# AllenNeuralDynamics/aind-exaspim-neuron-segmentation

Measured on AMD Instinct MI355X. Metric: affinity voxels/sec on 96^3 patches over a 1024x1024x1024 volume, 1 MI355X, higher is better.
Workload: dtype fp16; 1 GPU; 1024x1024x1024 uint16 volume, 96^3 patches, overlap 32, trim 8, batch 16, fp16 (IEEE half) storage of activations and weights / fp32 accumulate (BASELINE.json configs[2]); streams=1

## Files before the change

### aind_exaspim_neuron_segmentation_amd/_native.py

```python

import ctypes
import os

_HERE = os.path.dirname(os.path.abspath(__file__))
LIB_PATH = os.path.join(_HERE, "csrc", "libexaspim_affinity.so")

DT_F32, DT_BF16, DT_F16 = 0, 1, 2
VOX_U8, VOX_U16, VOX_I16, VOX_F32, VOX_F64 = 0, 1, 2, 3, 4
IN_F32, IN_PADDED_F32, IN_PADDED_SPLIT_F16, IN_PADDED_SPLIT_BF16 = 0, 1, 2, 3
UP_CONVT = 0x100
OPT_SEPARATE_POOL, OPT_SEPARATE_DEEP_POOLS, OPT_PLAIN_UPSAMPLE, OPT_FIRST_PER_GROUP = 1, 2, 4, 8
OPT_UPSAMPLE_PER_THREAD = 16

DTYPE_CODES = {
    "fp32": DT_F32, "float32": DT_F32, "f32": DT_F32,
    "bf16": DT_BF16, "bfloat16": DT_BF16,
    "fp16": DT_F16, "float16": DT_F16, "f16": DT_F16,
}


class Block(ctypes.Structure):

    _fields_ = [
        ("dims", ctypes.c_int32 * 3),
        ("origin", ctypes.c_int32 * 3),
        ("global_", ctypes.c_int32 * 3),
    ]

    @classmethod
    def make(cls, dims, origin=None, global_shape=None):
        origin = (0, 0, 0) if origin is None else origin
        global_shape = dims if global_shape is None else global_shape
        b = cls()
        b.dims[:] = [int(v) for v in dims]
        b.origin[:] = [int(v) for v in origin]
        b.global_[:] = [int(v) for v in global_shape]
        return b


class Window(ctypes.Structure):

    _fields_ = [
        ("patch", ctypes.c_int32 * 3),
        ("overlap", ctypes.c_int32 * 3),
        ("trim", ctypes.c_int32),
    ]

    @classmethod
    def make(cls, patch, overlap, trim):
        w = cls()
        w.patch[:] = [int(v) for v in patch]
        w.overlap[:] = [int(v) for v in overlap]
        w.trim = int(trim)
        return w


_lib = None

_I32x5 = ctypes.c_int32 * 5
_I32x3 = ctypes.c_int32 * 3
_vp = ctypes.c_void_p
_sz = ctypes.c_size_t
_i32 = ctypes.c_int32

SIGNATURES = {
# ... 86 lines not shown
```

### aind_exaspim_neuron_segmentation_amd/csrc/common.h

```cpp
#pragma once

#include <hip/hip_runtime.h>

#include <cstdarg>
#include <cstddef>
#include <cstdint>
#include <cstdio>

#include "../../include/exaspim_affinity.h"

namespace exaspim {

void set_error(const char* fmt, ...);
const char* get_error();

#define EXA_CHECK_ARG(cond, ...)                 \
    do {                                         \
        if (!(cond)) {                           \
            ::exaspim::set_error(__VA_ARGS__);   \
            return EXASPIM_E_INVALID;            \
        }                                        \
    } while (0)

#define EXA_CHECK_HIP(expr)                                                  \
// ... 68 lines not shown
    int cin_real = 0, cin = 0;
    int cout_real = 0, cout = 0;
    size_t w_off = 0;
    size_t b_off = 0;
    size_t p_off = 0;
};

struct UNetPlan {
    int channels[5] = {0, 0, 0, 0, 0};
    int out_channels = 0;
    int dtype = 0;
    bool convt = false;
    ConvTLayer up[4];
    int c0 = 0, c0p = 0;
    size_t first_p_off = 0;
    size_t first_w_off = 0;
    size_t first_b_off = 0;
    ConvLayer conv[kNumMfmaConvs];
    size_t head_p_off = 0;
    size_t head_w_off = 0;
    size_t head_b_off = 0;
    size_t packed_bytes = 0;
    size_t n_params = 0;
};

bool make_plan(const int32_t channels[5], int32_t out_channels, int32_t dtype,
               UNetPlan* plan);

int pack_weights(const UNetPlan& plan, const float* params, void* packed_host);

struct ConvArgs {
    const void* src_a;
    const void* src_b;
    int ca, cb;
    const void* weights;
    const void* weights_paired = nullptr;
    const void* weights_k32 = nullptr;
    const float* bias;
    void* dst;
    int cout;
    int n, d, h, w;
    float slope;
    const float* head_w = nullptr;
    const float* head_b = nullptr;
    float* head_out = nullptr;
    int head_oc = 0;
    int head_sigmoid = 0;
    int org[3] = {0, 0, 0};
    int ext[3] = {0, 0, 0};
    void* pool_dst = nullptr;
    float* partial = nullptr;
    size_t partial_patch_bytes = 0;
    int ksplit = 1;
#ifdef EXASPIM_TRACE
    unsigned long long* trace = nullptr;
#endif
};

int launch_conv3x3x3(int dtype, const ConvArgs& a, hipStream_t stream);
int launch_conv3x3x3_thin(int dtype, const ConvArgs& a, hipStream_t stream);
int conv_zcol_main_extent(int ext, int axis);
bool conv_can_fuse_head(int cout, int w, int head_oc);
bool conv_can_fuse_pool(int dtype, int cout, int d, int h, int w);

int launch_conv_first(int dtype, const float* x, float* xpad, const float* w, const float* bias,
                      void* dst, int n, int d, int h, int wd, int c0p, float slope,
                      hipStream_t stream, bool first_no_strips = false);
int launch_convt2(int dtype, const void* src, const void* weights, const float* bias, void* dst,
                  int n, int d, int h, int w, int cin, int cout, hipStream_t stream);
int launch_maxpool2(int dtype, const void* src, void* dst, int n, int d, int h, int w,
                    int c, hipStream_t stream);
int launch_upsample2(int dtype, const void* src, void* dst, int n, int d, int h, int w,
                     int c, int margin, hipStream_t stream, bool plain_kernel = false, bool per_thread = false);
int launch_absmax(int dtype, const void* src, size_t bytes, float* out, hipStream_t stream);
int launch_head(int dtype, const void* src, const float* w, const float* bias,
                float* out, int n, int d, int h, int wd, int c0p, int out_channels,
                int apply_sigmoid, hipStream_t stream);

}
```

### aind_exaspim_neuron_segmentation_amd/csrc/conv3d.hip

```cpp

#include <cstdlib>
#include <type_traits>

#include "common.h"

namespace exaspim {

typedef float f32x16 __attribute__((ext_vector_type(16)));
typedef float f32x4 __attribute__((ext_vector_type(4)));
typedef __bf16 bf16x8 __attribute__((ext_vector_type(8)));
typedef _Float16 f16x8 __attribute__((ext_vector_type(8)));

typedef unsigned int u32x4_t __attribute__((ext_vector_type(4)));

struct F32Tag { static constexpr int kG = 4; static constexpr int kCode = EXASPIM_DT_F32; };
struct BF16Tag { static constexpr int kG = 8; static constexpr int kCode = EXASPIM_DT_BF16; };
struct F16Tag { static constexpr int kG = 8; static constexpr int kCode = EXASPIM_DT_F16; };

template <typename Tag>
__device__ __forceinline__ void mma(f32x16& acc, const uint4& wf, const uint4& xf);

template <>
__device__ __forceinline__ void mma<F32Tag>(f32x16& acc, const uint4& wf, const uint4& xf) {
    acc = __builtin_amdgcn_mfma_f32_32x32x2f32(__uint_as_float(wf.x), __uint_as_float(xf.x), acc, 0, 0, 0);
// ... 1047 lines not shown
#if EXASPIM_BUFFER_STORES & 4
                    const __amdgpu_buffer_rsrc_t prsrc = make_rsrc(pplane, (size_t)CPT * pvox * 32);
#endif
#pragma unroll
                    for (int p0 = 0; p0 < NP; p0 += 64) {
                        const int p = p0 + lane_e;
#if EXASPIM_BUFFER_STORES & 4
                        const bool live0 = p < NP;
                        const int pc = live0 ? p : 0;
                        const int zp = pc / (8 * CPT * 2), rem = pc % (8 * CPT * 2);
                        const int ck = rem / 16, xp = (rem % 16) >> 1, sb = rem & 1;
                        const bool live = live0 && zb + 2 * zp + 1 < TZ;
                        const int zr = zb + 2 * zp + 1 < TZ ? zp : 0;
                        {
                            const char* rec = wl + (2 * zr) * (32 * RECP) + (2 * xp) * RECP + (ck * 2 + sb) * 16;
#else
                        const int zp = p / (8 * CPT * 2), rem = p % (8 * CPT * 2);
                        const int ck = rem / 16, xp = (rem % 16) >> 1, sb = rem & 1;
                        if (p < NP && zb + 2 * zp + 1 < TZ) {
                            const char* rec = wl + (2 * zp) * (32 * RECP) + (2 * xp) * RECP + (ck * 2 + sb) * 16;
#endif
                            uint4 m = *reinterpret_cast<const uint4*>(rec);
                            if (ES == 2) m = key16(m);
#pragma unroll
                            for (int k = 1; k < 8; ++k) {
                                const uint4 v = *reinterpret_cast<const uint4*>(
                                    rec + (k >> 2) * (32 * RECP) + ((k >> 1) & 1) * 16 * RECP + (k & 1) * RECP);
                                m = ES == 2 ? maxkey16(m, key16(v)) : max16<Tag>(m, v);
                            }
                            if (ES == 2) m = key16(m);
                            const int qz = (cur.z0 + zb) / 2 + zp, qy = cur.y0 / 2 + wave, qx = cur.x0 / 2 + xp;
#if EXASPIM_BUFFER_STORES & 4
                            const unsigned pvoff =
                                live && qz < pd && qy < ph && qx < pw2
                                    ? (unsigned)((ck * (int)pvox + (qz * ph + qy) * pw2 + qx) * 32 + sb * 16)
                                    : kOutOfRange;
                            buf_store16(m, prsrc, pvoff, 0u);
#else
                            if (qz < pd && qy < ph && qx < pw2)
                                *reinterpret_cast<uint4*>(pplane + ((size_t)ck * pvox +
                                                                    ((size_t)qz * ph + qy) * pw2 + qx) * 32 + sb * 16) = m;
#endif
                        }
                    }
                }
                __builtin_amdgcn_fence(__ATOMIC_ACQUIRE, "wavefront");
                __builtin_amdgcn_wave_barrier();
            }
        }
        EXA_TRACE(14);
        if (!has_next) break;
        if (!kLdsFreeEpilogue) __syncthreads();
        if (!(EXASPIM_STAGE_FIRST && kLdsFreeEpilogue)) stage_store();
        tile_id += t_step;
        cur = nxt;
    }
}

#ifdef EXASPIM_VARIANTS
template <int I, int N, typename F>
__device__ __forceinline__ void static_for(F&& f) {
    if constexpr (I < N) {
        f(std::integral_constant<int, I>{});
        static_for<I + 1, N>(f);
    }
}

template <typename Tag>
__device__ __forceinline__ void mma16(f32x4& acc, const uint4& wf, const uint4& xf);
template <>
__device__ __forceinline__ void mma16<BF16Tag>(f32x4& acc, const uint4& wf, const uint4& xf) {
    asm volatile("v_mfma_f32_16x16x32_bf16 %0, %1, %2, %0"
                 : "+v"(acc) : "v"(__builtin_bit_cast(u32x4, wf)), "v"(__builtin_bit_cast(u32x4, xf)));
}
template <>
__device__ __forceinline__ void mma16<F16Tag>(f32x4& acc, const uint4& wf, const uint4& xf) {
    asm volatile("v_mfma_f32_16x16x32_f16 %0, %1, %2, %0"
                 : "+v"(acc) : "v"(__builtin_bit_cast(u32x4, wf)), "v"(__builtin_bit_cast(u32x4, xf)));
}

template <typename Tag>
__device__ __forceinline__ void mma16_agpr(f32x4& acc, const uint4& wf, const uint4& xf);
template <>
__device__ __forceinline__ void mma16_agpr<BF16Tag>(f32x4& acc, const uint4& wf, const uint4& xf) {
    asm volatile("v_mfma_f32_16x16x32_bf16 %0, %1, %2, %0"
                 : "+a"(acc) : "v"(__builtin_bit_cast(u32x4, wf)), "v"(__builtin_bit_cast(u32x4, xf)));
}
template <>
__device__ __forceinline__ void mma16_agpr<F16Tag>(f32x4& acc, const uint4& wf, const uint4& xf) {
    asm volatile("v_mfma_f32_16x16x32_f16 %0, %1, %2, %0"
                 : "+a"(acc) : "v"(__builtin_bit_cast(u32x4, wf)), "v"(__builtin_bit_cast(u32x4, xf)));
}

template <typename Tag, int TZ, int TY, int MINW, int D, int HEAD = 0, bool POOL = false>
__global__ __launch_bounds__(TY * 16 * 2, MINW) void conv3x3x3_zpair(
    ConvArgs a, int tiles_z, int tiles_y, int tiles_x) {
    constexpr int TX = 16;
    constexpr int KC = 16, ES = 2;
    constexpr int HZ = TZ + 2, HY = TY + 2, HX = TX + 2;
    constexpr int HXP = HX;
    constexpr int PLANE = HY * HXP;
    constexpr int HVP = HZ * PLANE;
    constexpr int GS = (HVP + 15) / 16 * 16;
    constexpr int NWAVES = TY / 2;
    constexpr int NTHREADS = NWAVES * 64;
    constexpr int NPAIR = 2 * HY * HX;
// ... 557 lines not shown
                for (int ck = 0; ck < 4; ++ck) {
                    const uint4 val = *reinterpret_cast<const uint4*>(wl + vv * RECP + (ck * 2 + sub) * 16);
                    if (ok) *reinterpret_cast<uint4*>(dplane + ((size_t)ck * patch_vox + vox) * 32 + sub * 16) = val;
                }
                __builtin_amdgcn_fence(__ATOMIC_ACQUIRE, "wavefront");
                __builtin_amdgcn_wave_barrier();
            }
        }
        if (!more_tiles) break;
        tile = next;
    }
}

#endif

#ifdef EXASPIM_TRACE
int g_variant = 0;
#endif

static int resident_workgroups(int per_cu) {
    static int cus = 0;
    if (cus == 0) {
        int dev = 0, n = 0;
        if (hipGetDevice(&dev) != hipSuccess ||
            hipDeviceGetAttribute(&n, hipDeviceAttributeMultiprocessorCount, dev) != hipSuccess || n <= 0)
            n = 256;
        cus = n;
    }
    return cus * per_cu;
}

template <typename Tag, int TZ, int TY, int TX, int MINW, int D, int HEAD = 0, bool POOL = false>
static int launch_zpipe(const ConvArgs& a, hipStream_t stream) {
    const int tz = (a.ext[0] + TZ - 1) / TZ, ty = (a.ext[1] + TY - 1) / TY, tx = (a.ext[2] + TX - 1) / TX;
    const long long blocks = (long long)tz * ty * tx * a.n;
    if (blocks <= 0 || blocks > 0x7fffffffLL) {
        set_error("conv: grid of %lld blocks out of range", blocks);
        return EXASPIM_E_INVALID;
    }
    const int slices = a.cout / 32;
    long long wgs = resident_workgroups(MINW) / slices / 8 * 8;
    if (wgs < 8) wgs = 8;
    if (wgs > blocks) wgs = blocks;
#ifdef EXASPIM_TRACE
    if (g_variant >= 10 && g_variant < 20) wgs = blocks;
    if (const char* e = getenv("EXASPIM_TRACE_WGS_PER_CU")) wgs = resident_workgroups(1) * (long long)atoi(e) / slices / 8 * 8;
#endif
    dim3 grid((unsigned)wgs, slices);
    conv3x3x3_zpipe<Tag, TZ, TY, TX, MINW, D, HEAD, POOL><<<grid, TY * TX * 2, 0, stream>>>(a, tz, ty, tx);
    EXA_CHECK_HIP(hipGetLastError());
    return EXASPIM_OK;
}

#ifdef EXASPIM_VARIANTS
template <typename Tag, int TZ, int D, int HEAD = 0, bool POOL = false>
static int launch_zpair(const ConvArgs& a, hipStream_t stream) {
    constexpr int TY = 8, TX = 16, MINW = 2;
    const int tz = (a.ext[0] + TZ - 1) / TZ, ty = (a.ext[1] + TY - 1) / TY, tx = (a.ext[2] + TX - 1) / TX;
    const long long blocks = (long long)tz * ty * tx * a.n;
    if (blocks <= 0 || blocks > 0x7fffffffLL) {
        set_error("conv: grid of %lld blocks out of range", blocks);
        return EXASPIM_E_INVALID;
    }
    const int slices = a.cout / 32;
    long long wgs = resident_workgroups(MINW) / slices / 8 * 8;
    if (wgs < 8) wgs = 8;
    if (wgs > blocks) wgs = blocks;
    dim3 grid((unsigned)wgs, slices);
    conv3x3x3_zpair<Tag, TZ, TY, MINW, D, HEAD, POOL><<<grid, TY * TX * 2, 0, stream>>>(a, tz, ty, tx);
    EXA_CHECK_HIP(hipGetLastError());
    return EXASPIM_OK;
}

template <typename Tag, int TZ>
static int launch_zpair_head(const ConvArgs& a, hipStream_t stream) {
    if (a.head_out && a.cout == 32) {
        switch (a.head_oc) {
            case 1: return launch_zpair<Tag, TZ, 4, 1>(a, stream);
            case 2: return launch_zpair<Tag, TZ, 4, 2>(a, stream);
            case 3: return launch_zpair<Tag, TZ, 4, 3>(a, stream);
            case 4: return launch_zpair<Tag, TZ, 4, 4>(a, stream);
        }
    }
    if (a.pool_dst) return launch_zpair<Tag, TZ, 4, 0, true>(a, stream);
    return launch_zpair<Tag, TZ, 4>(a, stream);
}

template <typename Tag> struct HasPaired { static constexpr bool value = true; };
template <> struct HasPaired<F32Tag> { static constexpr bool value = false; };

static bool paired_enabled() {
    static int on = -1;
    if (on < 0) {
        const char* e = getenv("EXASPIM_ZPAIR");
        on = e && e[0] == '1';
    }
    return on != 0;
}

#endif

template <typename Tag>
__global__ __launch_bounds__(256) void splitk_reduce_kernel(const float* __restrict__ partial,
                                                            const float* __restrict__ bias,
                                                            void* __restrict__ dst, size_t nvox_all,
                                                            size_t patch_vox, int cout, int ksplit,
// ... 58 lines not shown
    }
    EXA_CHECK_HIP(hipGetLastError());
    if (b.ksplit > 1) {
        const size_t items = nvox_all * (a.cout / 4);
        splitk_reduce_kernel<Tag><<<(unsigned)((items + 255) / 256), 256, 0, stream>>>(
            a.partial, a.bias, a.dst, nvox_all, (size_t)a.d * a.h * a.w, a.cout, b.ksplit, a.slope);
        EXA_CHECK_HIP(hipGetLastError());
        if (POOL)
            return launch_maxpool2(Tag::kCode, a.dst, a.pool_dst, a.n, a.d, a.h, a.w, a.cout, stream);
    }
    return EXASPIM_OK;
}

template <typename Tag> struct ES_of { static constexpr int value = 16 / Tag::kG; };

template <typename Tag, int TZ, int TY, int TX, int WAVES_M, int WAVES_N, int MT, int NT, int MINW>
static int launch_cfg_pool(const ConvArgs& a, hipStream_t stream) {
    if constexpr (ES_of<Tag>::value == 2) {
        if (a.pool_dst)
            return launch_cfg<Tag, TZ, TY, TX, WAVES_M, WAVES_N, MT, NT, MINW, 3, false, false, true>(a, stream);
    }
    return launch_cfg<Tag, TZ, TY, TX, WAVES_M, WAVES_N, MT, NT, MINW>(a, stream);
}

template <typename Tag, int TZ, int D>
static int launch_zpipe_head(const ConvArgs& a, hipStream_t stream) {
    if (a.head_out && a.cout == 32) {
        switch (a.head_oc) {
            case 1: return launch_zpipe<Tag, TZ, 8, 16, 2, D, 1>(a, stream);
            case 2: return launch_zpipe<Tag, TZ, 8, 16, 2, D, 2>(a, stream);
            case 3: return launch_zpipe<Tag, TZ, 8, 16, 2, D, 3>(a, stream);
            case 4: return launch_zpipe<Tag, TZ, 8, 16, 2, D, 4>(a, stream);
        }
    }
    if (a.pool_dst) return launch_zpipe<Tag, TZ, 8, 16, 2, D, 0, true>(a, stream);
    return launch_zpipe<Tag, TZ, 8, 16, 2, D>(a, stream);
}

template <typename Tag, int TZ>
static int launch_zpipe_d(const ConvArgs& a, hipStream_t stream) {
#ifdef EXASPIM_TRACE
    if (g_variant % 10 == 3) return launch_zpipe_head<Tag, TZ, 3>(a, stream);
    if (g_variant % 10 == 5) return launch_zpipe_head<Tag, TZ, 5>(a, stream);
#endif
    return launch_zpipe_head<Tag, TZ, 4>(a, stream);
}

template <typename Tag>
static int launch_typed(const ConvArgs& a, hipStream_t stream) {
    if (a.w >= 16 && a.w % 16 == 0) {
#ifdef EXASPIM_TRACE
        if (g_variant >= 20) return launch_zpipe_d<Tag, 6>(a, stream);
#endif
        if (a.cout % 64 != 0) {
#ifdef EXASPIM_VARIANTS
            if constexpr (HasPaired<Tag>::value) {
                if (a.weights_paired && paired_enabled()) {
                    if (a.d % 6 == 0) return launch_zpair_head<Tag, 6>(a, stream);
                    return launch_zpair_head<Tag, 4>(a, stream);
                }
            }
#endif
#if EXASPIM_HEAD_TZ
            if (a.head_out && a.cout == 32 && a.ext[0] % 6 != 0 && a.ext[0] % EXASPIM_HEAD_TZ == 0) {
                switch (a.head_oc) {
                    case 1: return launch_zpipe<Tag, EXASPIM_HEAD_TZ, 8, 16, 2, 4, 1>(a, stream);
                    case 2: return launch_zpipe<Tag, EXASPIM_HEAD_TZ, 8, 16, 2, 4, 2>(a, stream);
                    case 3: return launch_zpipe<Tag, EXASPIM_HEAD_TZ, 8, 16, 2, 4, 3>(a, stream);
                    case 4: return launch_zpipe<Tag, EXASPIM_HEAD_TZ, 8, 16, 2, 4, 4>(a, stream);
                }
            }
#endif
            if (a.d % 6 == 0) return launch_zpipe_d<Tag, 6>(a, stream);
            return launch_zpipe_d<Tag, 4>(a, stream);
        }
#ifdef EXASPIM_VARIANTS
        if constexpr (HasPaired<Tag>::value) {
            static int t16 = -1;
            if (t16 < 0) { const char* e = getenv("EXASPIM_T16"); t16 = e && e[0] == '1'; }
            const bool whole = a.ext[0] == a.d && a.ext[1] == a.h && a.ext[2] == a.w;
            if (t16 && !a.pool_dst && a.weights_k32 && whole && a.cout == 64 && a.ca % 32 == 0 && a.cb % 32 == 0) {
                const int tz = cdiv(a.d, 4), ty = cdiv(a.h, 8), tx = cdiv(a.w, 16);
                const int ntiles = tz * ty * tx * a.n;
                long long nwg = resident_workgroups(1) / 8 * 8;
                if (nwg < 8) nwg = 8;
                if (nwg > ntiles) nwg = (ntiles + 7) / 8 * 8;
                conv3x3x3_t16<Tag, 2><<<(unsigned)nwg, 256, 0, stream>>>(a, tz, ty, tx);
                EXA_CHECK_HIP(hipGetLastError());
                return EXASPIM_OK;
            }
        }
#endif
#ifndef EXASPIM_T14_DMA
#define EXASPIM_T14_DMA 0
#endif
        if (a.pool_dst) return launch_cfg_pool<Tag, 4, 8, 16, 4, 1, 4, 2, 2>(a, stream);
        return launch_cfg<Tag, 4, 8, 16, 4, 1, 4, 2, 2, 3, false, EXASPIM_T14_DMA != 0>(a, stream);
    }
    if (a.w > 12) {
        if (a.cout % 64 == 0) return launch_cfg_pool<Tag, 4, 4, 24, 4, 1, 3, 2, 2>(a, stream);
        return launch_cfg_pool<Tag, 4, 4, 24, 4, 1, 3, 1, 2>(a, stream);
    }
    if (a.w > 6) {
        if (a.cout % 256 == 0) return launch_cfg_pool<Tag, 4, 4, 12, 2, 1, 3, 1, 2>(a, stream);
        if (a.cout % 128 == 0) return launch_cfg_pool<Tag, 4, 4, 12, 2, 2, 3, 2, 2>(a, stream);
        if (a.cout % 64 == 0) return launch_cfg_pool<Tag, 4, 4, 12, 2, 2, 3, 1, 2>(a, stream);
// ... 94 lines not shown
```

### aind_exaspim_neuron_segmentation_amd/csrc/engine.hip

```cpp

#include <algorithm>
#include <cstdlib>
#include <new>
#include <string_view>

#include "common.h"

namespace exaspim {

constexpr float kLeakySlope = 0.01f;

struct Workspace {
    size_t skip[5], a[5], b[5];
    size_t xpad;
    size_t bytes;
};

}

struct LayerTimer {
    static constexpr int kRing = 16384;
    uint32_t mask = 0;
    int next = 0, used = 0;
    hipEvent_t start[kRing], stop[kRing];
// ... 52 lines not shown
    if (workspace_bytes < ws.bytes) {
        set_error("forward: workspace %zu bytes < required %zu", workspace_bytes, ws.bytes);
        return EXASPIM_E_WORKSPACE;
    }
    char* base = static_cast<char*>(workspace);
    auto skip = [&](int l) { return (void*)(base + ws.skip[l]); };
    auto A = [&](int l) { return (void*)(base + ws.a[l]); };
    auto B = [&](int l) { return (void*)(base + ws.b[l]); };
    const int dt = p.dtype;
    int rc;

    const bool fuse_head = !absmax && conv_can_fuse_head(p.conv[kNumMfmaConvs - 1].cout, w, p.out_channels);
    const bool trimmed = fuse_head && trim > 0 && 2 * trim < d && 2 * trim < h && 2 * trim < w;
    const bool separate_pool = (e->options & EXASPIM_OPT_SEPARATE_POOL) != 0;
    const bool separate_deep = (e->options & EXASPIM_OPT_SEPARATE_DEEP_POOLS) != 0;
    bool fuse_pool[4];
    for (int l = 0; l < 4; ++l)
        fuse_pool[l] = !separate_pool && !(separate_deep && l > 0) && conv_can_fuse_pool(p.dtype, p.conv[2 * l].cout, d >> l, h >> l, w >> l);
    auto conv = [&](int idx, const void* sa, const void* sb, void* dst, int l) -> int {
        const ConvLayer& L = p.conv[idx];
        ConvArgs a;
        a.partial = reinterpret_cast<float*>(base + ws.xpad);
        a.partial_patch_bytes = (size_t)(d + 2) * (h + 2) * (w + 2) * sizeof(float);
        if (idx <= 6 && idx % 2 == 0 && fuse_pool[idx / 2]) a.pool_dst = A(idx / 2 + 1);
        const int margin = !trimmed ? 0 : idx == kNumMfmaConvs - 1 ? trim : idx == kNumMfmaConvs - 2 ? trim - 1 : 0;
        const int full[3] = {d >> l, h >> l, w >> l};
        for (int i = 0; i < 3; ++i) {
            a.org[i] = margin;
            a.ext[i] = full[i] - 2 * margin;
        }
        int rem_y = 0, rem_x = 0;
        const bool has_head = idx == kNumMfmaConvs - 1 && fuse_head;
        if (margin > 0 && !has_head && L.cout % 64 != 0 && full[2] % 16 == 0) {
            rem_y = a.ext[1] - conv_zcol_main_extent(a.ext[1], 1);
            rem_x = a.ext[2] - conv_zcol_main_extent(a.ext[2], 2);
            a.ext[1] -= rem_y;
            a.ext[2] -= rem_x;
        }
        if (idx == kNumMfmaConvs - 1 && fuse_head) {
            a.head_w = reinterpret_cast<const float*>(e->packed + p.head_w_off);
            a.head_b = reinterpret_cast<const float*>(e->packed + p.head_b_off);
            a.head_out = out;
            a.head_oc = p.out_channels;
            a.head_sigmoid = apply_sigmoid;
        }
        a.src_a = sa; a.src_b = sb; a.ca = L.ca; a.cb = L.cb;
        a.weights = e->packed + L.w_off;
        a.weights_paired = L.w2_off ? e->packed + L.w2_off : nullptr;
        a.weights_k32 = L.w3_off ? e->packed + L.w3_off : nullptr;
        a.bias = reinterpret_cast<const float*>(e->packed + L.b_off);
        a.dst = dst; a.cout = L.cout;
        a.n = n; a.d = d >> l; a.h = h >> l; a.w = w >> l;
        a.slope = kLeakySlope;
        LayerTimer* t = e->timer;
        const bool timed = t && (t->mask >> idx & 1u) && t->used < LayerTimer::kRing;
        int slot = 0;
        if (timed) {
            slot = t->next;
            EXA_CHECK_HIP(hipEventRecord(t->start[slot], stream));
        }
        int r = launch_conv3x3x3(dt, a, stream);
        if (timed && r == EXASPIM_OK) {
            EXA_CHECK_HIP(hipEventRecord(t->stop[slot], stream));
            t->layer[slot] = idx;
            t->next = (slot + 1) % LayerTimer::kRing;
            t->used++;
        }
        if (r == EXASPIM_OK && rem_y > 0) {
            ConvArgs b = a;
            b.org[1] = a.org[1] + a.ext[1]; b.ext[1] = rem_y;
            b.ext[2] = a.ext[2] + rem_x;
            r = launch_conv3x3x3_thin(dt, b, stream);
        }
        if (r == EXASPIM_OK && rem_x > 0) {
            ConvArgs b = a;
            b.org[2] = a.org[2] + a.ext[2]; b.ext[2] = rem_x;
            r = launch_conv3x3x3_thin(dt, b, stream);
        }
        if (r == EXASPIM_OK && absmax)
            r = launch_absmax(dt, dst, (size_t)n * (d >> l) * (h >> l) * (w >> l) * L.cout * dtype_size(dt),
                              absmax + 1 + idx, stream);
        return r;
    };
#define RUN(expr) do { rc = (expr); if (rc) return rc; } while (0)

    RUN(launch_conv_first(dt, x, x ? reinterpret_cast<float*>(base + ws.xpad)
                                   : const_cast<float*>(static_cast<const float*>(x_prepared)),
                          reinterpret_cast<const float*>(e->packed + p.first_w_off),
                          reinterpret_cast<const float*>(e->packed + p.first_b_off), A(0), n, d,
                          h, w, p.c0p, kLeakySlope, stream, (e->options & EXASPIM_OPT_FIRST_PER_GROUP) != 0));
    if (absmax) RUN(launch_absmax(dt, A(0), (size_t)n * d * h * w * p.c0p * dtype_size(dt), absmax, stream));
    RUN(conv(0, A(0), nullptr, skip(0), 0));
    for (int l = 1; l <= 4; ++l) {
        const ConvLayer& L0 = p.conv[2 * l - 1];
        const void* prev = skip(l - 1);
        if (!fuse_pool[l - 1])
            RUN(launch_maxpool2(dt, prev, A(l), n, d >> (l - 1), h >> (l - 1), w >> (l - 1), L0.ca,
                                stream));
        RUN(conv(2 * l - 1, A(l), nullptr, B(l), l));
        RUN(conv(2 * l, B(l), nullptr, l < 4 ? skip(l) : A(l), l));
    }
    const void* prev = A(4);
    for (int l = 3; l >= 0; --l) {
        const int i0 = 9 + 2 * (3 - l);
        const ConvLayer& L0 = p.conv[i0];
        if (p.convt) {
// ... 162 lines not shown
        case EXASPIM_DT_F32: return EXASPIM_IN_PADDED_F32;
        case EXASPIM_DT_F16: return EXASPIM_IN_PADDED_SPLIT_F16;
        case EXASPIM_DT_BF16: return EXASPIM_IN_PADDED_SPLIT_BF16;
    }
    return EXASPIM_E_INVALID;
}

extern "C" int exaspim_unet_forward_prepared(exaspim_unet* h, const void* x_prepared_dev, float* out_dev,
                                             int32_t n, int32_t d, int32_t hgt, int32_t w,
                                             int32_t apply_sigmoid, int32_t trim,
                                             void* workspace_dev, size_t workspace_bytes,
                                             void* stream) {
    EXA_CHECK_ARG(h && x_prepared_dev && out_dev && workspace_dev, "forward: NULL pointer");
    EXA_CHECK_ARG(n > 0, "forward: empty batch");
    EXA_CHECK_ARG(trim >= 0, "forward: negative trim %d", trim);
    EXA_CHECK_ARG(level_dims_ok(d, hgt, w),
                  "forward: patch %dx%dx%d: every dimension must be a positive multiple of 16",
                  d, hgt, w);
    return forward(h, nullptr, out_dev, n, d, hgt, w, apply_sigmoid, trim, workspace_dev,
                   workspace_bytes, (hipStream_t)stream, x_prepared_dev);
}

extern "C" int exaspim_unet_forward_trimmed(exaspim_unet* h, const float* x_dev, float* out_dev,
                                            int32_t n, int32_t d, int32_t hgt, int32_t w,
                                            int32_t apply_sigmoid, int32_t trim,
                                            void* workspace_dev, size_t workspace_bytes,
                                            void* stream) {
    EXA_CHECK_ARG(h && x_dev && out_dev && workspace_dev, "forward: NULL pointer");
    EXA_CHECK_ARG(n > 0, "forward: empty batch");
    EXA_CHECK_ARG(trim >= 0, "forward: negative trim %d", trim);
    EXA_CHECK_ARG(level_dims_ok(d, hgt, w),
                  "forward: patch %dx%dx%d: every dimension must be a positive multiple of 16",
                  d, hgt, w);
    return forward(h, x_dev, out_dev, n, d, hgt, w, apply_sigmoid, trim, workspace_dev,
                   workspace_bytes, (hipStream_t)stream);
}

extern "C" int exaspim_unet_forward_absmax(exaspim_unet* h, const float* x_dev, float* out_dev,
                                           int32_t n, int32_t d, int32_t hgt, int32_t w,
                                           int32_t apply_sigmoid, float* absmax_dev,
                                           void* workspace_dev, size_t workspace_bytes, void* stream) {
    EXA_CHECK_ARG(h && x_dev && out_dev && workspace_dev && absmax_dev, "forward_absmax: NULL pointer");
    EXA_CHECK_ARG(n > 0, "forward: empty batch");
    EXA_CHECK_ARG(level_dims_ok(d, hgt, w),
                  "forward: patch %dx%dx%d: every dimension must be a positive multiple of 16",
                  d, hgt, w);
    return forward(h, x_dev, out_dev, n, d, hgt, w, apply_sigmoid, 0, workspace_dev, workspace_bytes,
                   (hipStream_t)stream, nullptr, absmax_dev);
}

extern "C" int exaspim_unet_set_options(exaspim_unet* h, uint32_t options) {
    EXA_CHECK_ARG(h != nullptr, "set_options: NULL handle");
    EXA_CHECK_ARG((options & ~(uint32_t)(EXASPIM_OPT_SEPARATE_POOL | EXASPIM_OPT_SEPARATE_DEEP_POOLS | EXASPIM_OPT_PLAIN_UPSAMPLE | EXASPIM_OPT_FIRST_PER_GROUP |
                                          EXASPIM_OPT_UPSAMPLE_PER_THREAD)) == 0,
                  "set_options: unknown option bits 0x%x", options);
    h->options = options;
    return EXASPIM_OK;
}
```

### include/exaspim_affinity.h

```cpp
#ifndef EXASPIM_AFFINITY_H
#define EXASPIM_AFFINITY_H

#include <stddef.h>
#include <stdint.h>

#ifdef __cplusplus
extern "C" {
#endif

#define EXASPIM_ABI_VERSION 5

#define EXASPIM_OK 0
#define EXASPIM_E_INVALID (-1)
#define EXASPIM_E_HIP (-2)
#define EXASPIM_E_WORKSPACE (-3)
#define EXASPIM_E_NODEVICE (-4)

#define EXASPIM_DT_F32 0
#define EXASPIM_DT_BF16 1
#define EXASPIM_DT_F16 2
#define EXASPIM_UP_CONVT 0x100

#define EXASPIM_VOX_U8 0
#define EXASPIM_VOX_U16 1
// ... 14 lines not shown
    int32_t overlap[3];
    int32_t trim;
} exaspim_window;

int exaspim_abi_version(void);
const char* exaspim_last_error(void);


size_t exaspim_unet_param_count(const int32_t channels[5], int32_t out_channels,
                                int32_t dtype);

size_t exaspim_unet_packed_bytes(const int32_t channels[5], int32_t out_channels,
                                 int32_t dtype);

int exaspim_unet_pack_weights(const int32_t channels[5], int32_t out_channels,
                              int32_t dtype, const float* params, size_t n_params,
                              void* packed_host, size_t packed_bytes);

int exaspim_unet_create(const int32_t channels[5], int32_t out_channels,
                        int32_t dtype, int32_t device, const void* packed_dev,
                        size_t packed_bytes, exaspim_unet** out);
void exaspim_unet_destroy(exaspim_unet* h);

size_t exaspim_unet_workspace_bytes(const exaspim_unet* h, int32_t n, int32_t d,
                                    int32_t hgt, int32_t w);

int exaspim_unet_forward(exaspim_unet* h, const float* x_dev, float* out_dev,
                         int32_t n, int32_t d, int32_t hgt, int32_t w,
                         int32_t apply_sigmoid, void* workspace_dev,
                         size_t workspace_bytes, void* stream);

int exaspim_unet_forward_trimmed(exaspim_unet* h, const float* x_dev, float* out_dev,
                                 int32_t n, int32_t d, int32_t hgt, int32_t w,
                                 int32_t apply_sigmoid, int32_t trim, void* workspace_dev,
                                 size_t workspace_bytes, void* stream);

int exaspim_unet_input_layout(const exaspim_unet* h);
int exaspim_unet_forward_prepared(exaspim_unet* h, const void* x_prepared_dev, float* out_dev,
                                  int32_t n, int32_t d, int32_t hgt, int32_t w,
                                  int32_t apply_sigmoid, int32_t trim, void* workspace_dev,
                                  size_t workspace_bytes, void* stream);

#define EXASPIM_ABSMAX_SLOTS 22
int exaspim_unet_forward_absmax(exaspim_unet* h, const float* x_dev, float* out_dev,
                                int32_t n, int32_t d, int32_t hgt, int32_t w,
                                int32_t apply_sigmoid, float* absmax_dev, void* workspace_dev,
                                size_t workspace_bytes, void* stream);

#define EXASPIM_OPT_SEPARATE_POOL 1u
#define EXASPIM_OPT_SEPARATE_DEEP_POOLS 2u
#define EXASPIM_OPT_PLAIN_UPSAMPLE 4u
#define EXASPIM_OPT_FIRST_PER_GROUP 8u
#define EXASPIM_OPT_UPSAMPLE_PER_THREAD 16u
int exaspim_unet_set_options(exaspim_unet* h, uint32_t options);

int exaspim_unet_timing_begin(exaspim_unet* h, uint32_t conv_mask);
int exaspim_unet_timing_read(exaspim_unet* h, double ms_sum[17], int32_t count[17]);


int exaspim_histogram(const void* vol_dev, int32_t vox_dtype, size_t n,
                      double clip, int32_t has_clip, int32_t pass,
                      uint32_t prefix, uint64_t* hist_dev, void* stream);

int exaspim_histogram_wide(const void* vol_dev, int32_t vox_dtype, size_t n,
                           double clip, int32_t has_clip, int32_t pass,
                           uint64_t prefix, uint64_t* hist_dev, void* stream);

#define EXASPIM_IN_F32 0
#define EXASPIM_IN_PADDED_F32 1
#define EXASPIM_IN_PADDED_SPLIT_F16 2
#define EXASPIM_IN_PADDED_SPLIT_BF16 3
int exaspim_gather_patches_as(const void* vol_dev, int32_t vox_dtype,
                              const exaspim_block* blk, const int32_t* starts_dev,
                              int32_t n, const int32_t patch[3], double clip,
                              int32_t has_clip, double mn, double denom, int32_t layout,
                              void* out_dev, void* stream);
int exaspim_gather_patches(const void* vol_dev, int32_t vox_dtype,
                           const exaspim_block* blk, const int32_t* starts_dev,
                           int32_t n, const int32_t patch[3], double clip,
                           int32_t has_clip, double mn, double denom,
                           float* out_dev, void* stream);


int exaspim_stitch_accumulate(const float* pred_dev, const int32_t* starts_dev,
                              int32_t n, int32_t channels,
                              const exaspim_window* win, float* accum_dev,
                              const exaspim_block* blk, void* stream);

int exaspim_stitch_finalize(float* accum_dev, int32_t channels,
                            const exaspim_window* win, const exaspim_block* blk,
                            void* stream);

int exaspim_export_f16(const float* src_dev, void* dst_dev, size_t n, void* stream);


int exaspim_synth_volume_u16(uint16_t* vol_dev, const exaspim_block* blk,
                             uint64_t seed, void* stream);

#ifdef __cplusplus
}
#endif
#endif
```

Measured before the change: 786.1 million voxels/s.

## Add dedicated two-chunk 32-channel conv kernel with fused head for final layer

Adds a specialized persistent 3x3x3 conv kernel (zcol2) for 16-bit 32-in/32-out layers that carry a fused output head. Both input channel chunks are staged in LDS at the same time. The next tile's loads and a ring of weight loads are interleaved with the MFMA steps. The kernel is used by default, and an option bit restores the old zpipe path. It aims to cut per-tile synchronization and load latency on the last decoder conv, at the cost of more LDS use and register pressure.

Result: no change. 786.7 million voxels/s, median of 6 (+0.1%).

```diff
diff --git a/aind_exaspim_neuron_segmentation_amd/_native.py b/aind_exaspim_neuron_segmentation_amd/_native.py
--- a/aind_exaspim_neuron_segmentation_amd/_native.py
+++ b/aind_exaspim_neuron_segmentation_amd/_native.py
@@ -11,6 +11,7 @@
 UP_CONVT = 0x100
 OPT_SEPARATE_POOL, OPT_SEPARATE_DEEP_POOLS, OPT_PLAIN_UPSAMPLE, OPT_FIRST_PER_GROUP = 1, 2, 4, 8
 OPT_UPSAMPLE_PER_THREAD = 16
+OPT_ZPIPE_TWO_CHUNK = 32
 
 DTYPE_CODES = {
     "fp32": DT_F32, "float32": DT_F32, "f32": DT_F32,
diff --git a/aind_exaspim_neuron_segmentation_amd/csrc/common.h b/aind_exaspim_neuron_segmentation_amd/csrc/common.h
--- a/aind_exaspim_neuron_segmentation_amd/csrc/common.h
+++ b/aind_exaspim_neuron_segmentation_amd/csrc/common.h
@@ -144,6 +144,7 @@
     float* partial = nullptr;
     size_t partial_patch_bytes = 0;
     int ksplit = 1;
+    bool zpipe_two_chunk = false;
 #ifdef EXASPIM_TRACE
     unsigned long long* trace = nullptr;
 #endif
diff --git a/aind_exaspim_neuron_segmentation_amd/csrc/conv3d.hip b/aind_exaspim_neuron_segmentation_amd/csrc/conv3d.hip
--- a/aind_exaspim_neuron_segmentation_amd/csrc/conv3d.hip
+++ b/aind_exaspim_neuron_segmentation_amd/csrc/conv3d.hip
@@ -1123,6 +1123,284 @@
         if (!has_next) break;
         if (!kLdsFreeEpilogue) __syncthreads();
         if (!(EXASPIM_STAGE_FIRST && kLdsFreeEpilogue)) stage_store();
+        tile_id += t_step;
+        cur = nxt;
+    }
+}
+
+template <typename Tag, int TZ, int TY, int TX, int MINW, int D, int PD, int HEAD>
+__global__ __launch_bounds__(TY* TX * 2, MINW) void conv3x3x3_zcol2(
+    ConvArgs a, int tiles_z, int tiles_y, int tiles_x) {
+    constexpr int G = Tag::kG;
+    constexpr int KC = 2 * G;
+    constexpr int ES = 16 / G;
+    static_assert(ES == 2 && HEAD >= 1 && HEAD <= 4, "16-bit storage types, fused head");
+    constexpr int HZ = TZ + 2, HY = TY + 2, HX = TX + 2;
+    constexpr int HXP = HX;
+    constexpr int PLANE = HY * HXP;
+    constexpr int HVP = HZ * PLANE;
+    constexpr int GS = HVP + (24 - HVP % 16) % 16;
+    constexpr int CS = 2 * GS;
+    constexpr int NWAVES = TY * TX / 32;
+    constexpr int NTHREADS = NWAVES * 64;
+    constexpr int NPAIR = 2 * HY * HX;
+    constexpr int REM = NPAIR > NTHREADS ? NPAIR - NTHREADS : 0;
+    constexpr int SEC = (REM * HZ + NTHREADS - 1) / NTHREADS;
+    constexpr int NITEMS = HZ + SEC;
+    constexpr int NST = 2 * NITEMS;
+    constexpr int NS = 9 * HZ;
+    constexpr int NSS = 2 * NS;
+    constexpr int R = D + 1;
+    constexpr int NT = 18;
+#ifndef EXASPIM_ZCOL2_LOAD_STRIDE
+#define EXASPIM_ZCOL2_LOAD_STRIDE 4
+#endif
+    constexpr int LOAD_STRIDE = NSS / NST >= EXASPIM_ZCOL2_LOAD_STRIDE ? EXASPIM_ZCOL2_LOAD_STRIDE : NSS / NST;
+    static_assert(TY * TX % 32 == 0 && NPAIR <= 2 * NTHREADS && LOAD_STRIDE >= 1, "tile shape");
+    static_assert(PD >= 1 && PD < NT && NT % (PD + 1) == 0, "weight ring depth (the ring wraps from tile to tile)");
+
+    __shared__ __attribute__((aligned(16))) uint4 lds[2 * CS];
+
+    const int tid = threadIdx.x;
+    const int lane = tid & 63;
+    const int wave = __builtin_amdgcn_readfirstlane(tid >> 6);
+    const int half = lane >> 5;
+    const int r = (TX == 16 && (lane & 16)) ? 16 + (((lane & 15) - HXP) & 15) : (lane & 31);
+
+    const int total = tiles_z * tiles_y * tiles_x * a.n;
+    int t_first, t_count, t_step;
+    {
+        const int q = total >> 3, rem = total & 7;
+        const int xcd = blockIdx.x & 7, slot = blockIdx.x >> 3;
+        t_first = (xcd < rem ? xcd * (q + 1) : rem * (q + 1) + (xcd - rem) * q) + slot;
+        t_count = q + (xcd < rem ? 1 : 0) - slot;
+        t_step = (gridDim.x + 7 - xcd) >> 3;
+    }
+    if (t_count <= 0) return;
+
+    struct Tile {
+        int z0, y0, x0, nb;
+    };
+    auto tile_at = [&](int id) {
+        Tile t;
+        t.x0 = __builtin_amdgcn_readfirstlane(a.org[2] + (id % tiles_x) * TX); id /= tiles_x;
+        t.y0 = __builtin_amdgcn_readfirstlane(a.org[1] + (id % tiles_y) * TY); id /= tiles_y;
+        t.z0 = __builtin_amdgcn_readfirstlane(a.org[0] + (id % tiles_z) * TZ); id /= tiles_z;
+        t.nb = __builtin_amdgcn_readfirstlane(id);
+        return t;
+    };
+
+    const int pos = wave * 32 + r;
+    const int col = (pos / TX) * HXP + (pos % TX) + half * GS;
+
+    const int plane_vox = a.h * a.w;
+    const size_t patch_vox = (size_t)a.d * plane_vox;
+    unsigned p_voff;
+    unsigned s_voff[SEC > 0 ? SEC : 1];
+    auto set_offsets = [&](const Tile& t) {
+        const int ft = wave * 64 + fresh_lane();
+        {
+            const int p_hy = (ft >> 1) / HX, p_hx = (ft >> 1) % HX, p_kg = ft & 1;
+            const int gy = t.y0 + p_hy - 1, gx = t.x0 + p_hx - 1;
+            const bool in = ft < NPAIR && (unsigned)gy < (unsigned)a.h && (unsigned)gx < (unsigned)a.w;
+            p_voff = in ? (unsigned)(gy * a.w + gx) * 32u + p_kg * 16u : kOutOfRange;
+        }
+#pragma unroll
+        for (int k = 0; k < SEC; ++k) {
+            const int q = ft + k * NTHREADS;
+            const int pr = NTHREADS + q % REM, hz = q / REM;
+            const int c = pr >> 1, kg = pr & 1;
+            const int gz = t.z0 + hz - 1, gy = t.y0 + c / HX - 1, gx = t.x0 + c % HX - 1;
+            const bool in = q < REM * HZ && (unsigned)gz < (unsigned)a.d &&
+                            (unsigned)gy < (unsigned)a.h && (unsigned)gx < (unsigned)a.w;
+            s_voff[k] = in ? (unsigned)((gz * a.h + gy) * a.w + gx) * 32u + kg * 16u : kOutOfRange;
+        }
+    };
+
+    __shared__ __attribute__((aligned(16))) float bias_s[32];
+    if (tid < 32) bias_s[tid] = a.bias[tid];
+    __shared__ __attribute__((aligned(16))) float head_s[HEAD * 32 + 4];
+    if (tid < HEAD * 32) head_s[tid] = a.head_w[tid];
+    if (tid < HEAD) head_s[HEAD * 32 + tid] = a.head_b[tid];
+
+    const __amdgpu_buffer_rsrc_t wrsrc = make_rsrc(a.weights, (size_t)2 * 27 * 1024);
+    const unsigned wvoff = (unsigned)lane * 16u;
+    auto wsoff = [](int tap, int dz) {
+        return (unsigned)(((tap / 9) * 27 + dz * 9 + tap % 9) * 1024);
+    };
+
+    struct ChunkSrc {
+        __amdgpu_buffer_rsrc_t rsrc;
+        __amdgpu_buffer_rsrc_t none;
+        unsigned cbase;
+    };
+    auto chunk_src = [&](int c, int nb) {
+        const char* src;
+        int cs, ch0;
+        if (c * KC < a.ca) {
+            src = static_cast<const char*>(a.src_a); cs = a.ca; ch0 = c * KC;
+        } else {
+            src = static_cast<const char*>(a.src_b); cs = a.cb; ch0 = c * KC - a.ca;
+        }
+        const size_t patchb = patch_vox * cs * ES;
+        return ChunkSrc{make_rsrc(src + (size_t)nb * patchb, patchb), make_rsrc(src + (size_t)nb * patchb, 0),
+                        (unsigned)(ch0 / KC) * (unsigned)patch_vox * 32u};
+    };
+    uint4 stg[NST];
+    auto load_piece = [&](const ChunkSrc& cs, int z0, int i) {
+        if (i < HZ) {
+            const int gz = z0 + i - 1;
+            return (unsigned)gz < (unsigned)a.d ? buf_load16(cs.rsrc, p_voff, cs.cbase + (unsigned)gz * plane_vox * 32u)
+                                                : buf_load16(cs.none, p_voff, 0);
+        }
+        return buf_load16(cs.rsrc, s_voff[i - HZ], cs.cbase);
+    };
+    auto stage_store = [&]() {
+        const int ft = wave * 64 + fresh_lane();
+        const int p_slot = (ft & 1) * GS + ((ft >> 1) / HX) * HXP + (ft >> 1) % HX;
+#pragma unroll
+        for (int c = 0; c < 2; ++c) {
+            if (ft < NPAIR) {
+#pragma unroll
+                for (int hz = 0; hz < HZ; ++hz) lds[c * CS + p_slot + hz * PLANE] = stg[c * NITEMS + hz];
+            }
+#pragma unroll
+            for (int k = 0; k < SEC; ++k) {
+                const int q = ft + k * NTHREADS;
+                const int pr = NTHREADS + q % REM, hz = q / REM;
+                const int cc = pr >> 1, kg = pr & 1;
+                if (q < REM * HZ) lds[c * CS + kg * GS + hz * PLANE + (cc / HX) * HXP + cc % HX] = stg[c * NITEMS + HZ + k];
+            }
+        }
+    };
+
+    int tile_id = t_first;
+    Tile cur = tile_at(tile_id);
+    set_offsets(cur);
+    {
+        const ChunkSrc c0 = chunk_src(0, cur.nb), c1 = chunk_src(1, cur.nb);
+#pragma unroll
+        for (int i = 0; i < NITEMS; ++i) {
+            stg[i] = load_piece(c0, cur.z0, i);
+            stg[NITEMS + i] = load_piece(c1, cur.z0, i);
+        }
+    }
+    uint4 wr[PD + 1][3];
+#pragma unroll
+    for (int t = 0; t < PD; ++t)
+#pragma unroll
+        for (int dz = 0; dz < 3; ++dz) wr[t][dz] = buf_load16(wrsrc, wvoff, wsoff(t, dz));
+    stage_store();
+
+    for (;;) {
+        __syncthreads();
+        f32x16 acc[TZ];
+        const int half_t = fresh_lane() >> 5;
+#pragma unroll
+        for (int q = 0; q < 4; ++q) {
+            const float4 b = *reinterpret_cast<const float4*>(bias_s + 8 * q + 4 * half_t);
+#pragma unroll
+            for (int mt = 0; mt < TZ; ++mt) {
+                acc[mt][4 * q + 0] = b.x; acc[mt][4 * q + 1] = b.y;
+                acc[mt][4 * q + 2] = b.z; acc[mt][4 * q + 3] = b.w;
+            }
+        }
+
+        t_count -= t_step;
+        const bool has_next = t_count > 0;
+        const Tile nxt = has_next ? tile_at(tile_id + t_step) : cur;
+        set_offsets(nxt);
+        const ChunkSrc n0 = chunk_src(0, nxt.nb), n1 = chunk_src(1, nxt.nb);
+
+        auto operand = [&](int S) {
+            const int c = S / NS, g = (S % NS) / HZ, zin = S % HZ;
+            return lds[c * CS + col + zin * PLANE + (g / 3) * HXP + g % 3];
+        };
+        uint4 xr[R];
+#pragma unroll
+        for (int S = 0; S < D; ++S) xr[S % R] = operand(S);
+        __builtin_amdgcn_sched_barrier(0);
+        if (EXASPIM_SETPRIO) __builtin_amdgcn_s_setprio(EXASPIM_SETPRIO);
+        auto chunk_steps = [&](auto chunk) {
+            constexpr int c = decltype(chunk)::value;
+#pragma unroll
+            for (int s = 0; s < NS; ++s) {
+                const int S = c * NS + s;
+                const int t = S / HZ, zin = S % HZ;
+                if (S + D < NSS) xr[(S + D) % R] = operand(S + D);
+                if (zin == 0) {
+#pragma unroll
+                    for (int dz = 0; dz < 3; ++dz)
+                        wr[(t + PD) % (PD + 1)][dz] = buf_load16(wrsrc, wvoff, wsoff((t + PD) % NT, dz));
+                }
+                if (S % LOAD_STRIDE == 0 && S / LOAD_STRIDE < NST) {
+                    const int j = S / LOAD_STRIDE;
+                    stg[j] = j < NITEMS ? load_piece(n0, nxt.z0, j) : load_piece(n1, nxt.z0, j - NITEMS);
+                }
+#pragma unroll
+                for (int dz = 0; dz < 3; ++dz) {
+                    const int z = zin - dz;
+                    if (z >= 0 && z < TZ) mma_inplace<Tag>(acc[z], wr[t % (PD + 1)][dz], xr[S % R]);
+                }
+                __builtin_amdgcn_sched_barrier(0);
+            }
+        };
+        chunk_steps(std::integral_constant<int, 0>{});
+        chunk_steps(std::integral_constant<int, 1>{});
+        if (EXASPIM_SETPRIO) __builtin_amdgcn_s_setprio(0);
+        asm volatile("s_nop 7\n\ts_nop 7\n\ts_nop 1");
+        __syncthreads();
+        {
+#pragma unroll
+            for (int i = 0; i < NST; ++i)
+                asm volatile("" : "+v"(stg[i].x), "+v"(stg[i].y), "+v"(stg[i].z), "+v"(stg[i].w));
+        }
+
+        const int lane_e = fresh_lane();
+        const int half_e = lane_e >> 5;
+        const int r_e = (TX == 16 && (lane_e & 16)) ? 16 + (((lane_e & 15) - HXP) & 15) : (lane_e & 31);
+        const int pos_e = wave * 32 + r_e;
+        const int gy = cur.y0 + pos_e / TX, gx = cur.x0 + pos_e % TX;
+        const bool okyx = gy < a.org[1] + a.ext[1] && gx < a.org[2] + a.ext[2];
+        float part[TZ][HEAD];
+#pragma unroll
+        for (int z = 0; z < TZ; ++z)
+#pragma unroll
+            for (int o = 0; o < HEAD; ++o) part[z][o] = 0.f;
+#pragma unroll
+        for (int q = 0; q < 4; ++q) {
+            float4 hw[HEAD];
+#pragma unroll
+            for (int o = 0; o < HEAD; ++o)
+                hw[o] = *reinterpret_cast<const float4*>(head_s + o * 32 + 8 * q + 4 * half_e);
+#pragma unroll
+            for (int z = 0; z < TZ; ++z) {
+                const float v0 = leaky(acc[z][4 * q + 0], a.slope), v1 = leaky(acc[z][4 * q + 1], a.slope);
+                const float v2 = leaky(acc[z][4 * q + 2], a.slope), v3 = leaky(acc[z][4 * q + 3], a.slope);
+#pragma unroll
+                for (int o = 0; o < HEAD; ++o)
+                    part[z][o] = fmaf(v3, hw[o].w, fmaf(v2, hw[o].z, fmaf(v1, hw[o].y, fmaf(v0, hw[o].x, part[z][o]))));
+            }
+        }
+        const size_t plane = (size_t)a.h * a.w;
+        float* const hpatch = a.head_out + (size_t)cur.nb * HEAD * a.d * plane;
+        const size_t hbytes = (size_t)HEAD * a.d * plane * sizeof(float);
+        const unsigned hvoff[2] = {okyx && half_e == 0 ? (unsigned)(gy * a.w + gx) * 4u : kOutOfRange,
+                                   okyx && half_e == 1 ? (unsigned)(gy * a.w + gx) * 4u : kOutOfRange};
+#pragma unroll
+        for (int z = 0; z < TZ; ++z) {
+            const int gz = cur.z0 + z;
+            const __amdgpu_buffer_rsrc_t hrsrc = make_rsrc(hpatch, gz < a.org[0] + a.ext[0] ? hbytes : (size_t)0);
+#pragma unroll
+            for (int o = 0; o < HEAD; ++o) {
+                float v = part[z][o] + __shfl_xor(part[z][o], 32) + head_s[HEAD * 32 + o];
+                if (a.head_sigmoid) v = 1.f / (1.f + expf(-v));
+                __builtin_amdgcn_raw_buffer_store_b32(__float_as_uint(v), hrsrc, (int)hvoff[o & 1],
+                                                      (int)((unsigned)(o * a.d + gz) * (unsigned)plane * 4u), 0);
+            }
+        }
+        if (!has_next) break;
+        stage_store();
         tile_id += t_step;
         cur = nxt;
     }
@@ -1786,6 +2064,23 @@
     return EXASPIM_OK;
 }
 
+template <typename Tag, int HEAD>
+static int launch_zcol2(const ConvArgs& a, hipStream_t stream) {
+    constexpr int TZ = 4, TY = 8, TX = 16, MINW = 2;
+    const int tz = (a.ext[0] + TZ - 1) / TZ, ty = (a.ext[1] + TY - 1) / TY, tx = (a.ext[2] + TX - 1) / TX;
+    const long long blocks = (long long)tz * ty * tx * a.n;
+    if (blocks <= 0 || blocks > 0x7fffffffLL) {
+        set_error("conv: grid of %lld blocks out of range", blocks);
+        return EXASPIM_E_INVALID;
+    }
+    long long wgs = resident_workgroups(MINW) / 8 * 8;
+    if (wgs < 8) wgs = 8;
+    if (wgs > blocks) wgs = blocks;
+    conv3x3x3_zcol2<Tag, TZ, TY, TX, MINW, 4, 2, HEAD><<<dim3((unsigned)wgs, 1), TY * TX * 2, 0, stream>>>(a, tz, ty, tx);
+    EXA_CHECK_HIP(hipGetLastError());
+    return EXASPIM_OK;
+}
+
 #ifdef EXASPIM_VARIANTS
 template <typename Tag, int TZ, int D, int HEAD = 0, bool POOL = false>
 static int launch_zpair(const ConvArgs& a, hipStream_t stream) {
@@ -1950,6 +2245,16 @@
 #ifdef EXASPIM_TRACE
         if (g_variant >= 20) return launch_zpipe_d<Tag, 6>(a, stream);
 #endif
+        if constexpr (ES_of<Tag>::value == 2) {
+            if (!a.zpipe_two_chunk && a.head_out && a.cout == 32 && a.ca + a.cb == 32) {
+                switch (a.head_oc) {
+                    case 1: return launch_zcol2<Tag, 1>(a, stream);
+                    case 2: return launch_zcol2<Tag, 2>(a, stream);
+                    case 3: return launch_zcol2<Tag, 3>(a, stream);
+                    case 4: return launch_zcol2<Tag, 4>(a, stream);
+                }
+            }
+        }
         if (a.cout % 64 != 0) {
 #ifdef EXASPIM_VARIANTS
             if constexpr (HasPaired<Tag>::value) {
diff --git a/aind_exaspim_neuron_segmentation_amd/csrc/engine.hip b/aind_exaspim_neuron_segmentation_amd/csrc/engine.hip
--- a/aind_exaspim_neuron_segmentation_amd/csrc/engine.hip
+++ b/aind_exaspim_neuron_segmentation_amd/csrc/engine.hip
@@ -128,6 +128,7 @@
         a.dst = dst; a.cout = L.cout;
         a.n = n; a.d = d >> l; a.h = h >> l; a.w = w >> l;
         a.slope = kLeakySlope;
+        a.zpipe_two_chunk = (e->options & EXASPIM_OPT_ZPIPE_TWO_CHUNK) != 0;
         LayerTimer* t = e->timer;
         const bool timed = t && (t->mask >> idx & 1u) && t->used < LayerTimer::kRing;
         int slot = 0;
@@ -396,7 +397,7 @@
 extern "C" int exaspim_unet_set_options(exaspim_unet* h, uint32_t options) {
     EXA_CHECK_ARG(h != nullptr, "set_options: NULL handle");
     EXA_CHECK_ARG((options & ~(uint32_t)(EXASPIM_OPT_SEPARATE_POOL | EXASPIM_OPT_SEPARATE_DEEP_POOLS | EXASPIM_OPT_PLAIN_UPSAMPLE | EXASPIM_OPT_FIRST_PER_GROUP |
-                                          EXASPIM_OPT_UPSAMPLE_PER_THREAD)) == 0,
+                                          EXASPIM_OPT_UPSAMPLE_PER_THREAD | EXASPIM_OPT_ZPIPE_TWO_CHUNK)) == 0,
                   "set_options: unknown option bits 0x%x", options);
     h->options = options;
     return EXASPIM_OK;
diff --git a/include/exaspim_affinity.h b/include/exaspim_affinity.h
--- a/include/exaspim_affinity.h
+++ b/include/exaspim_affinity.h
@@ -90,6 +90,7 @@
 #define EXASPIM_OPT_PLAIN_UPSAMPLE 4u
 #define EXASPIM_OPT_FIRST_PER_GROUP 8u
 #define EXASPIM_OPT_UPSAMPLE_PER_THREAD 16u
+#define EXASPIM_OPT_ZPIPE_TWO_CHUNK 32u
 int exaspim_unet_set_options(exaspim_unet* h, uint32_t options);
 
 int exaspim_unet_timing_begin(exaspim_unet* h, uint32_t conv_mask);
```
